# aperezhortal/pySPEEDY

Hardware: AMD Instinct MI355X
Metric: simulated-years/day (whole node), T30L8 (higher is better)
Workload: dtype f64

## Files before the change

pyspeedy_amd/csrc/capi.hip:

```cpp
#include <hip/hip_runtime.h>

#include <cstdio>
#include <cstring>
#include <mutex>
#include <string>
#include <vector>

#include "../../include/pyspeedy_amd.h"
#include "context.hpp"
#include "device_tables.hpp"
#include "surface_host.hpp"
#include "triangle.hpp"
#include "vertical_consts.hpp"

namespace spd {
hipError_t run_spec2grid(const DeviceTables &T, int stage, const double *src, double *dst, int kcos, int nfields,
                         hipStream_t stream);
hipError_t run_grid2spec(const DeviceTables &T, int stage, const double *src, double *dst, int prescale, int nfields,
                         hipStream_t stream);
hipError_t run_vort2vel(const DeviceTables &T, const double *vor, const double *div, double *ucos, double *vcos,
                        int nfields, hipStream_t s);
hipError_t run_vel2vort(const DeviceTables &T, const double *ucos, const double *vcos, double *vor, double *div,
                        int nfields, hipStream_t s);
hipError_t run_gradient(const DeviceTables &T, const double *psi, double *psdx, double *psdy, int nfields, hipStream_t s);
// ... 255 lines not shown
    else if (s == "ifac") { tmp.assign(t.ifac.begin(), t.ifac.end()); arr(tmp); }
    else if (s == "tri_packed") {
        tmp.assign(1 + NSPEC, -1.0);
        tmp[0] = tri::kPacked;
        for (int n = 0; n < NX; ++n)
            for (int m = 0; m < MX; ++m)
                if (tri::fwd_filled(m, n)) tmp[1 + n * MX + m] = tri::packed_index(m, n);
        arr(tmp);
    }
    else if (s == "tri_inv_needed") {
        tmp.assign(NSPEC, 0.0);
        for (int n = 0; n < NX; ++n)
            for (int m = 0; m < MX; ++m) tmp[n * MX + m] = tri::inv_needed(m, n) ? 1.0 : 0.0;
        arr(tmp);
    }
    else return fail(SPD_E_ARG, "spd_get_table_host: unknown table '" + s + "'");
    if (buf) {
        if (buf_elems < n) return fail(SPD_E_SIZE, "spd_get_table_host: buffer too small for '" + s + "'");
        std::memcpy(buf, src, n * sizeof(double));
    }
    return static_cast<long>(n);
}

int spd_calendar_walk(int year, int month, int day, int hour, int minute, int nsteps, int32_t *ymdhm, int32_t *month_idx,
                      int32_t *imont1, double *tmonth, double *tyear) {
    if (nsteps < 0 || month < 1 || month > 12 || day < 1 || day > 31) return fail(SPD_E_ARG, "spd_calendar_walk: bad start date or step count");
    Calendar c;
    c.set(year, month, day, hour, minute);
    for (int s = 0;; ++s) {
        if (ymdhm) {
// ... 160 lines not shown
```

pyspeedy_amd/csrc/dynamics.hip:

```cpp
#include <hip/hip_runtime.h>

#include <type_traits>

#include "coupler_point.hpp"
#include "device_tables.hpp"
#include "diagnostics_block.hpp"
#include "dyn_column.hpp"
#include "launch_events.hpp"
#include "model.hpp"
#include "sppt_point.hpp"

namespace spd {

namespace {
using d2 = double __attribute__((ext_vector_type(2)));
constexpr int NG = IX * IL;
constexpr int kT = 256;

__device__ constexpr double CPd = 1004.0f;
__device__ constexpr double AKAPd = 2.0f / 7.0f;
__device__ constexpr double RGASd = AKAPd * CPd;
__device__ constexpr double WILd = 0.53f, TDRSd = 24.0f * 30.0f;

__device__ inline d2 times_i(d2 z) { return d2{-z.y, z.x}; }
// ... 28 lines not shown
        rb = d2{-cm * s.bp.x + cp * s.bn.x + zp.x, -cm * s.bp.y + cp * s.bn.y + zp.y};
    }
}
}

namespace {
__device__ __forceinline__ d2 geo_up(d2 ph_below, d2 t_below, d2 t_here, double xg2_below, double xg1_here) {
    return d2{fma(xg1_here, t_here.x, fma(xg2_below, t_below.x, ph_below.x)),
              fma(xg1_here, t_here.y, fma(xg2_below, t_below.y, ph_below.y))};
}
__device__ __forceinline__ d2 geo_corr(d2 ph, d2 t_below, d2 t_above, double corf) {
    return d2{fma(corf, t_below.x - t_above.x, ph.x), fma(corf, t_below.y - t_above.y, ph.y)};
}
}

template <bool SPPT>
__global__ __launch_bounds__(kT) void geopotential_kernel(ModelPtrs P, DynDeviceTables D, int first, int count, int tl, SpptArgs sp) {
    const int ngeo = (count * NSPEC + kT - 1) / kT;
    if (SPPT && static_cast<int>(blockIdx.x) >= ngeo) {
        sppt_update_point(sp, static_cast<long>(blockIdx.x - ngeo) * kT + threadIdx.x);
        return;
    }
    const int gid = blockIdx.x * kT + threadIdx.x;
    if (gid >= count * NSPEC) return;
    const int lm = gid / NSPEC, mem = first + lm, k = gid - lm * NSPEC, m = k % MX;
    const d2 *t = reinterpret_cast<const d2 *>(P.t) + (static_cast<size_t>(mem) * 2 + tl) * 8 * NSPEC + k;
    d2 *phi = reinterpret_cast<d2 *>(P.phi) + static_cast<size_t>(mem) * 8 * NSPEC + k;
    d2 tt[KX], ph[KX];
#pragma unroll
    for (int l = 0; l < KX; ++l) tt[l] = t[static_cast<size_t>(l) * NSPEC];
    const d2 phis = reinterpret_cast<const d2 *>(P.phis)[static_cast<size_t>(mem) * NSPEC + k];
    ph[KX - 1] = d2{fma(D.xgeop1[KX - 1], tt[KX - 1].x, phis.x), fma(D.xgeop1[KX - 1], tt[KX - 1].y, phis.y)};
#pragma unroll
    for (int l = KX - 2; l >= 0; --l) ph[l] = geo_up(ph[l + 1], tt[l + 1], tt[l], D.xgeop2[l + 1], D.xgeop1[l]);
    if (m == 0) {
#pragma unroll
        for (int l = 1; l < KX - 1; ++l) ph[l] = geo_corr(ph[l], tt[l + 1], tt[l - 1], D.geo_corf[l]);
    }
#pragma unroll
    for (int l = 0; l < KX; ++l) phi[static_cast<size_t>(l) * NSPEC] = ph[l];
// ... 20 lines not shown
    double r = a[0];
#pragma unroll
    for (int i = 1; i < N; ++i) r = (l == i) ? a[i] : r;
    return r;
}
template <int N>
__device__ inline d2 pick(const d2 (&a)[N], int l) {
    d2 r = a[0];
#pragma unroll
    for (int i = 1; i < N; ++i) r = (l == i) ? a[i] : r;
    return r;
}
}

struct NoCoupler {};
template <bool FOLD, bool EARLY, typename CA>
__global__ __launch_bounds__(kT) void spectral_step_kernel(ModelPtrs P, DeviceTables T, DynDeviceTables D, int M, int first,
                                                           int count, int j1, double dt, double eps, CA cpl) {
    int nblocks = gridDim.x;
    if constexpr (std::is_same<CA, CouplerArgs>::value) {
        nblocks = (count * NSPEC * KX + kT - 1) / kT;
        if (static_cast<int>(blockIdx.x) >= nblocks) {
            const int gid = (blockIdx.x - nblocks) * kT + threadIdx.x;
            if (gid < cpl.count * NG) {
                const int lm = gid / NG;
                coupler_point(cpl.S, cpl.first + lm, gid - lm * NG, cpl.w, cpl.day, cpl.land_coupling, cpl.sst_anomaly,
                              cpl.anom_planes, cpl.fresh);
            }
            return;
        }
    }
    const int xcd = blockIdx.x & 7, q = nblocks >> 3, r = nblocks & 7;
    const int block = xcd * q + (xcd < r ? xcd : r) + (blockIdx.x >> 3);
    const int gid = block * kT + threadIdx.x;
    const int w = gid >> 6, lane = gid & 63;
    if (w >= count * kCoefBlocks) return;
    const int l = lane >> 3, kk = lane & 7;
    const int lm = w / kCoefBlocks, mem = first + lm, k = (w - lm * kCoefBlocks) * 8 + kk, n = k / MX, m = k - n * MX;
    const size_t f8 = static_cast<size_t>(mem) * 8 * NSPEC;
    const size_t fo = static_cast<size_t>(l) * NSPEC;
    const size_t tf = (static_cast<size_t>(mem) * 8 + l) * tri::kPacked;
    const size_t pair = static_cast<size_t>(M) * 8 * tri::kPacked;
    const d2 *su = reinterpret_cast<const d2 *>(P.specu) + tf, *sv = reinterpret_cast<const d2 *>(P.specv) + tf;
    const d2 *ske = reinterpret_cast<const d2 *>(P.spec_ke) + tf, *stt_f = reinterpret_cast<const d2 *>(P.spec_tt) + tf;
    const d2 *str_f = reinterpret_cast<const d2 *>(P.spec_tr) + tf;
    const d2 *sps = reinterpret_cast<const d2 *>(P.spec_ps) + static_cast<size_t>(mem) * tri::kPacked;
    const PackedAt at = packed_at(m, n);
    const double el2 = T.el2[k];
    d2 vordt, divdt, tdt, trdt, dump;
    const size_t s0 = static_cast<size_t>(mem) * 2 * 8 * NSPEC + fo + k;
    const size_t lvl = static_cast<size_t>(8) * NSPEC;
    d2 *vorS = reinterpret_cast<d2 *>(P.vor) + s0, *divS = reinterpret_cast<d2 *>(P.div) + s0;
    d2 *tS = reinterpret_cast<d2 *>(P.t) + s0, *trS = reinterpret_cast<d2 *>(P.tr) + s0;
// ... 15 lines not shown
            s_uv.ap = su[at.p], s_uv.bp = sv[at.p];
            s_ut.ap = su[pair + at.p], s_ut.bp = sv[pair + at.p];
            s_uq.ap = su[2 * pair + at.p], s_uq.bp = sv[2 * pair + at.p];
        }
        if (at.has_n) {
            s_uv.an = su[at.n], s_uv.bn = sv[at.n];
            s_ut.an = su[pair + at.n], s_ut.bn = sv[pair + at.n];
            s_uq.an = su[2 * pair + at.n], s_uq.bn = sv[2 * pair + at.n];
        }
    };
    auto load_diffusion = [&]() {
        dmp = D.dmp[k], dmp1 = D.dmp1[k], dmpd = D.dmpd[k], dmp1d = D.dmp1d[k], dmps = D.dmps[k], dmp1s = D.dmp1s[k];
        trf = T.trfilt[k];
        tcorh = reinterpret_cast<const d2 *>(P.tcorh)[static_cast<size_t>(mem) * NSPEC + k];
        qcorh = reinterpret_cast<const d2 *>(P.qcorh)[static_cast<size_t>(mem) * NSPEC + k];
    };
    if constexpr (EARLY) {
        load_tendencies(true);
        ph = reinterpret_cast<const d2 *>(P.phi)[f8 + fo + k];
        div1 = divS[0];
        ps1 = psS[0];
        const double *xj = D.xj + static_cast<size_t>(KX) * KX * (l_tot > 0 ? l_tot - 1 : 0);
#pragma unroll
        for (int k1 = 0; k1 < KX; ++k1) xc_l[k1] = D.xc[l + KX * k1], xj_l[k1] = xj[l + KX * k1], xd_l[k1] = D.xd[l + KX * k1];
        elz = D.elz[k];
        load_diffusion();
        vor1 = vorS[0], t1 = tS[0], tr1 = trS[0];
        vor2 = vorS[lvl], div2 = divS[lvl], t2 = tS[lvl], tr2 = trS[lvl], ps2 = psS[NSPEC];
        if (FOLD) phis_k = reinterpret_cast<const d2 *>(P.phis)[static_cast<size_t>(mem) * NSPEC + k];
        apply_stencil<1>(s_uv, k, m, n, T, vordt, divdt);
// ... 39 lines not shown
        double dtr_l = 0.0, dtr_l1 = 0.0;
#pragma unroll
        for (int j = 1; j < KX; ++j) {
            const double d = D.tref[j] - D.tref[j - 1];
            dtr_l = (l == j) ? d : dtr_l;
            dtr_l1 = (l + 1 == j) ? d : dtr_l1;
        }
        const d2 dumk_l = d2{sig_l.x * dtr_l, sig_l.y * dtr_l}, dumk_l1 = d2{sig_l1.x * dtr_l1, sig_l1.y * dtr_l1};
        const double dhsr_l = pick(D.dhsr, l), tref3_l = pick(D.tref3, l), tref2_l = pick(D.tref2, l);
        tdt.x = tdt.x - (dumk_l1.x + dumk_l.x) * dhsr_l + tref3_l * (sig_l1.x + sig_l.x) - tref2_l * dmeanc.x;
        tdt.y = tdt.y - (dumk_l1.y + dumk_l.y) * dhsr_l + tref3_l * (sig_l1.y + sig_l.y) - tref2_l * dmeanc.y;
    }
    {
        if constexpr (!EARLY) ph = reinterpret_cast<const d2 *>(P.phi)[f8 + fo + k];
        const double c = RGASd * tref_l;
        const d2 x = d2{ph.x + c * ps1.x, ph.y + c * ps1.y};
        const d2 lap = d2{-x.x * el2, -x.y * el2};
        divdt = d2{divdt.x - lap.x, divdt.y - lap.y};
    }

    {
        d2 all[KX];
        gather_levels(tdt, kk, all);
        d2 ye{0.0, 0.0};
#pragma unroll
        for (int k1 = 0; k1 < KX; ++k1) {
            const double x = EARLY ? xd_l[k1] : D.xd[l + KX * k1];
            ye = d2{ye.x + x * all[k1].x, ye.y + x * all[k1].y};
        }
        if constexpr (!EARLY) elz = D.elz[k];
// ... 13 lines not shown
        gather_levels(divdt, kk, all);
#pragma unroll
        for (int j = 0; j < KX; ++j) psdt = d2{psdt.x - all[j].x * D.dhsx[j], psdt.y - all[j].y * D.dhsx[j]};
#pragma unroll
        for (int k1 = 0; k1 < KX; ++k1) {
            const double x = EARLY ? xc_l[k1] : D.xc[l + KX * k1];
            tdt = d2{tdt.x + x * all[k1].x, tdt.y + x * all[k1].y};
        }
    }

    if constexpr (!EARLY) load_diffusion();
    const double sdrag = 1.0f / (TDRSd * 3600.0f);
    auto diffuse = [](d2 field, d2 fdt, double a, double b) { return d2{(fdt.x - a * field.x) * b, (fdt.y - a * field.y) * b}; };
    auto advance = [&](d2 *base, size_t stride, d2 o1, d2 o2, d2 fdt) -> d2 {
        if (!EARLY) o1 = base[0], o2 = base[stride];
        fdt = d2{fdt.x * trf, fdt.y * trf};
        const d2 oj = (j1 == 0) ? o1 : o2;
        const d2 fnew = d2{o1.x + dt * fdt.x, o1.y + dt * fdt.y};
        const double we = WILd * eps;
        const d2 n1 = d2{oj.x + we * (o1.x - 2 * oj.x + fnew.x), oj.y + we * (o1.y - 2 * oj.y + fnew.y)};
        const d2 oja = (j1 == 0) ? n1 : oj;
        const double we2 = (1.0f - WILd) * eps;
        const d2 n2 = d2{fnew.x - we2 * (n1.x - 2.0f * oja.x + fnew.x), fnew.y - we2 * (n1.y - 2.0f * oja.y + fnew.y)};
        stream_store(&base[0], n1);
        stream_store(&base[stride], n2);
        return n1;
    };
    {
        if constexpr (!EARLY) vor1 = vorS[0], t1 = tS[0], tr1 = trS[0];
        d2 vd = diffuse(vor1, vordt, dmp, dmp1);
        d2 dd = diffuse(div1, divdt, dmpd, dmp1d);
        const double tcorv_l = pick(D.tcorv, l), qcorv_l = pick(D.qcorv, l);
        const d2 ct = d2{t1.x + tcorh.x * tcorv_l, t1.y + tcorh.y * tcorv_l};
        d2 td = diffuse(ct, tdt, dmp, dmp1);
        if (l == 0 && m == 0) {
            vd = d2{vd.x - sdrag * vor1.x, vd.y - sdrag * vor1.y};
            dd = d2{dd.x - sdrag * div1.x, dd.y - sdrag * div1.y};
        }
// ... 19 lines not shown
            if (m == 0 && l >= 1 && l < KX - 1) {
                d2 tb = tall[2], ta = tall[0];
                double corf = D.geo_corf[1];
#pragma unroll
                for (int j = 2; j < KX - 1; ++j) {
                    tb = (l == j) ? tall[j + 1] : tb;
                    ta = (l == j) ? tall[j - 1] : ta;
                    corf = (l == j) ? D.geo_corf[j] : corf;
                }
                pn = geo_corr(pn, tb, ta, corf);
            }
            stream_store(&reinterpret_cast<d2 *>(P.phi_next)[f8 + fo + k], pn);
        }
    }
    if (l == 0) advance(psS, NSPEC, ps1, ps2, psdt);
}

__global__ __launch_bounds__(64 * KX) void diagnostics_kernel(CheckArgs c, DeviceTables T) {
    diagnostics_block(c, T, c.first + static_cast<int>(blockIdx.x));
}

hipError_t run_geopotential(const ModelPtrs &P, const DynDeviceTables &D, int first, int count, int tl, const SpptArgs *sppt,
                            hipStream_t s) {
    const int ngeo = (count * NSPEC + kT - 1) / kT;
    if (sppt) {
        const long n = static_cast<long>(sppt->M) * KX * NSPEC;
        launch(geopotential_kernel<true>, dim3(ngeo + static_cast<unsigned>((n + kT - 1) / kT)), dim3(kT), 0, s, P, D,
                           first, count, tl, *sppt);
    } else {
        launch(geopotential_kernel<false>, dim3(ngeo), dim3(kT), 0, s, P, D, first, count, tl, SpptArgs{});
    }
    return hipGetLastError();
}
hipError_t run_dyn_grid(const ModelPtrs &P, const DynDeviceTables &D, int M, hipStream_t s) {
    launch(dyn_grid_kernel, dim3((M * NG + kT - 1) / kT), dim3(kT), 0, s, P, D, M);
    return hipGetLastError();
}
namespace {
template <bool FOLD, bool EARLY, typename CA>
void launch_spectral_step(dim3 grid, hipStream_t s, const ModelPtrs &P, const DeviceTables &T, const DynDeviceTables &D, int M,
                          int first, int count, int j1, double dt, double eps, const CA &cpl) {
    launch(spectral_step_kernel<FOLD, EARLY, CA>, grid, dim3(kT), 0, s, P, T, D, M, first, count, j1, dt, eps, cpl);
}
template <typename CA>
void dispatch_spectral_step(bool fold, bool early, dim3 grid, hipStream_t s, const ModelPtrs &P, const DeviceTables &T,
                            const DynDeviceTables &D, int M, int first, int count, int j1, double dt, double eps, const CA &cpl) {
    if (fold && early) launch_spectral_step<true, true, CA>(grid, s, P, T, D, M, first, count, j1, dt, eps, cpl);
    else if (fold) launch_spectral_step<true, false, CA>(grid, s, P, T, D, M, first, count, j1, dt, eps, cpl);
    else if (early) launch_spectral_step<false, true, CA>(grid, s, P, T, D, M, first, count, j1, dt, eps, cpl);
    else launch_spectral_step<false, false, CA>(grid, s, P, T, D, M, first, count, j1, dt, eps, cpl);
}
}
hipError_t run_spectral_step(const ModelPtrs &P, const DeviceTables &T, const DynDeviceTables &D, int M, int first, int count,
                             int j1, double dt, double eps, const CouplerArgs *cpl, bool early, hipStream_t s) {
    const int nspec = (count * NSPEC * KX + kT - 1) / kT;
    const bool fold = P.phi_next != nullptr;
    if (cpl)
        dispatch_spectral_step(fold, early, dim3(nspec + (cpl->count * NG + kT - 1) / kT), s, P, T, D, M, first, count, j1, dt, eps,
                               *cpl);
    else
        dispatch_spectral_step(fold, early, dim3(nspec), s, P, T, D, M, first, count, j1, dt, eps, NoCoupler{});
    return hipGetLastError();
}
hipError_t run_diagnostics(const ModelPtrs &P, const DeviceTables &T, int M, int tl, int *err, double *diag, int ticket,
                           hipStream_t s) {
    hipLaunchKernelGGL(diagnostics_kernel, dim3(M), dim3(64 * KX), 0, s, CheckArgs{P.vor, P.div, P.t, tl, err, diag, ticket}, T);
    return hipGetLastError();
}
hipError_t run_diagnostics_range(const ModelPtrs &P, const DeviceTables &T, int first, int count, int tl, int *err, double *diag,
                                 int ticket, hipStream_t s) {
    if (count <= 0) return hipSuccess;
    hipLaunchKernelGGL(diagnostics_kernel, dim3(count), dim3(64 * KX), 0, s, CheckArgs{P.vor, P.div, P.t, tl, err, diag, ticket, first}, T);
    return hipGetLastError();
}

}
// ... 1 lines not shown
```

pyspeedy_amd/csrc/model.hip:

```cpp
#include <dlfcn.h>
#include <hip/hip_runtime.h>

#include <algorithm>
#include <atomic>
#include <chrono>
#include <cmath>
#include <cstring>
#include <map>
#include <memory>
#include <mutex>
#include <string>
#include <thread>
#include <utility>
#include <vector>

#include "../../include/pyspeedy_amd.h"
#include "context.hpp"
#include "model.hpp"
#include "coupler_point.hpp"
#include "diagnostics_block.hpp"
#include "bounded_call.hpp"
#include "launch_events.hpp"
#include "sppt_point.hpp"
#include "plev.hpp"
#include "stats.hpp"
#include "spectra.hpp"
#include "tape.hpp"
#include "enstape.hpp"
#include "acctape.hpp"
#include "stream_apart.hpp"
#include "surface.hpp"

namespace spd {
hipError_t run_spec2grid_table(const DeviceTables &T, const FieldDesc *table, int nfields, hipStream_t st);
hipError_t run_grid2spec_table(const DeviceTables &T, const FieldDesc *table, int nfields, hipStream_t st);
hipError_t run_physics(const DeviceTables &T, const spd_physics_args &a, int nmembers, int fp32, hipStream_t s);
hipError_t run_dyn_physics(const ModelPtrs &P, const DynDeviceTables &D, const DeviceTables &T, const spd_physics_args &a,
                           int first, int nmembers, int fp32, int store32, int diag, hipStream_t s);
hipError_t run_geopotential(const ModelPtrs &P, const DynDeviceTables &D, int first, int count, int tl, const SpptArgs *sppt,
                            hipStream_t s);
hipError_t run_dyn_grid(const ModelPtrs &P, const DynDeviceTables &D, int M, hipStream_t s);
hipError_t run_spectral_step(const ModelPtrs &P, const DeviceTables &T, const DynDeviceTables &D, int M, int first, int count,
                             int j1, double dt, double eps, const CouplerArgs *cpl, bool early, hipStream_t s);
hipError_t run_diagnostics(const ModelPtrs &P, const DeviceTables &T, int M, int tl, int *err, double *diag, int ticket,
                           hipStream_t s);
hipError_t run_diagnostics_range(const ModelPtrs &P, const DeviceTables &T, int first, int count, int tl, int *err, double *diag,
                                 int ticket, hipStream_t s);
hipError_t run_coupler(const SurfacePtrs &S, int first, int count, const TimeInterp &w, int day, int land_coupling,
                       int sst_anomaly, int anom_planes, int fresh, hipStream_t s);
hipError_t run_forcing(const SurfacePtrs &S, int first, int count, const ZonalDevice &Z, double gamlat, double *corh_t,
                       double *corh_q, hipStream_t s);
hipError_t run_rest_state(const RestPtrs &R, int M, const RestConsts &c, hipStream_t s);
hipError_t run_scale_orog(const double *orog, double *phi0, long n, hipStream_t s);
hipError_t run_change_storage(double *array, long n, bool to_float, void *scratch, hipStream_t s);
hipError_t run_land_sea_init(const LandSeaPtrs &P, const LandSeaConsts &K, int first, int count, double *rows, hipStream_t s);
hipError_t run_multi_copy(const CopyList &L, hipStream_t s);
hipError_t run_spec2grid_table_check(const DeviceTables &T, const FieldDesc *table, int nfields, const CheckArgs &check, int members,
                                     hipStream_t st);
// ... 43 lines not shown
        char *base;
        size_t size, used;
    };
    std::vector<Block> blocks;
    std::map<std::string, RegEntry> reg;
    FieldDesc *inv_table[2][2] = {{nullptr, nullptr}, {nullptr, nullptr}};
    FieldDesc *inv_table_sppt[2][2] = {{nullptr, nullptr}, {nullptr, nullptr}};
    FieldDesc *inv_table32[2][2] = {{nullptr, nullptr}, {nullptr, nullptr}}, *inv_table_sppt32[2][2] = {{nullptr, nullptr}, {nullptr, nullptr}};
    FieldDesc *fwd_table = nullptr;
    double *phi_buf[2] = {nullptr, nullptr};
    int phi_cur = 0;
    bool phi_ahead = false, fold_geo = true;
    bool groups_apart = true;
    int *d_err = nullptr;
    double *d_diag = nullptr;
    int *h_err[2] = {nullptr, nullptr}, *h_err_sync = nullptr;
    hipEvent_t err_event[2] = {nullptr, nullptr};
    int next_slot = 0;
    bool slot_busy[2] = {false, false};
    int check_ticket = 0, slot_ticket[2] = {0, 0};
    struct DeferredCheck {
        bool active = false;
        int slot = -1, time_level = 2;
        hipStream_t stream = nullptr;
    } deferred;
    hipStream_t slot_stream[2] = {nullptr, nullptr};
    bool slot_rode[2] = {false, false};
    int checks_alone = 0, checks_rode = 0;
    double air_absortivity_co2 = 6.0;
    SurfacePtrs S{};
// ... 516 lines not shown
    for (const char *name : {"t_grid_phys", "q_grid_phys", "phi_grid_phys", "pslg_phys", "u_grid_phys", "v_grid_phys",
                             "tt_rsw", "rad_tau2", "rad_strat_corr",
                             "rad_st4a", "rad_flux", "precnv", "precls", "cbmf", "slrd", "slr", "olr", "slru", "ustr", "vstr"})
        m->reg[name].f32 = true;
    if (rc == SPD_OK) {
        const spd_dyn_tables *base = nullptr;
        rc = dyn_tables(h, 0.0, nullptr, &base);
        if (rc == SPD_OK) m->D = base->dev;
    }
    if (rc == SPD_OK) {
        void *p = nullptr;
        rc = arena_alloc(m, sizeof(int) * M, &p);
        m->d_err = static_cast<int *>(p);
        if (rc == SPD_OK) rc = arena_alloc(m, sizeof(double) * M * 24, &p);
        m->d_diag = static_cast<double *>(p);
    }
    if (rc == SPD_OK) rc = build_tables(m);
    if (rc != SPD_OK) {
        spd_model_destroy(m);
        return rc;
    }
    *out = m;
    return SPD_OK;
}

int spd_model_destroy(spd_model_handle m) {
    if (!m) return SPD_OK;
    (void)hipSetDevice(m->ctx->device);
    constexpr size_t kIdleBytes = static_cast<size_t>(1) << 30;
    bool keep_first = false;
// ... 193 lines not shown
    m->P.phi = m->phi_buf[m->phi_cur];
    m->P.phi_next = m->fold_geo ? m->phi_buf[m->phi_cur ^ 1] : nullptr;
    m->reg["phi"].ptr = m->P.phi;
    m->phi_ahead = m->fold_geo;
    return !ahead;
}

static void sppt_advance(spd_model *m) {
    if (!m->sppt_on) return;
    m->sppt_first = false;
    m->sppt_step += 1;
}

static hipError_t step_range(spd_model *m, int j1, int j2, double dt, int compute_shortwave, int first, int count, int diag,
                             bool run_geo, const CouplerArgs *cpl, hipStream_t s, hipEvent_t after_grid2spec = nullptr,
                             const CheckArgs *ride = nullptr) {
    const DeviceTables &T = m->ctx->dev;
    const int M = m->M;
    hipError_t e = hipSuccess;
    if (m->fail_launch_after >= 0 && m->fail_launch_after-- == 0) return hipErrorLaunchFailure;
    SpptArgs sp{};
    if (m->sppt_on)
        sp = sppt_args(m->sppt_spec + static_cast<size_t>(first) * 8 * NSPEC * C, T, count, m->sppt_seed, m->sppt_member_base + first,
                       m->sppt_step, m->sppt_first ? 1 : 0);
    if (run_geo) {
        ProfScope ps(m, SPD_K_GEOPOTENTIAL, count, s);
        e = run_geopotential(m->P, m->D, first, count, 0, m->sppt_on ? &sp : nullptr, s);
    } else if (m->sppt_on) {
        ProfScope ps(m, SPD_K_SPPT, 8 * count, s);
        e = run_sppt_update(sp, s);
    }
    spd_physics_args pa = m->pa;
    pa.compute_shortwave = compute_shortwave ? 1 : 0;
    pa.air_absortivity_co2 = m->air_absortivity_co2;
    pa.sppt_pattern = m->sppt_on ? m->sppt_grid : nullptr;
    if (e == hipSuccess) {
        const int per = m->inv_per_member + (m->sppt_on ? 8 : 0);
        FieldDesc *table = (m->stored32 ? (m->sppt_on ? m->inv_table_sppt32 : m->inv_table32)
                                         : (m->sppt_on ? m->inv_table_sppt : m->inv_table))[j2 - 1][m->phi_cur];
        ProfScope ps(m, SPD_K_SPEC2GRID, per * count, s);
        if (m->deferred.active && first == 0 && count == M && s == m->deferred.stream) {
            const int slot = m->deferred.slot;
// ... 21 lines not shown
            }
        } else {
            ProfScope ps(m, compute_shortwave ? SPD_K_COLUMN_SW : SPD_K_COLUMN, count, s);
            e = run_dyn_physics(m->P, m->D, T, pa, first, count, m->phys_fp32, m->stored32 ? 1 : 0, diag, s);
        }
    }
    if (e == hipSuccess) {
        ProfScope ps(m, SPD_K_GRID2SPEC, 73 * count, s);
        e = run_grid2spec_table(T, m->fwd_table + static_cast<size_t>(first) * 73, 73 * count, s);
    }
    if (after_grid2spec && e == hipSuccess) e = hipEventRecord(after_grid2spec, s);
    const double eps = (j1 == 1) ? 0.0 : static_cast<double>(0.05f);
    if (e == hipSuccess) {
        ProfScope ps(m, SPD_K_SPECTRAL_STEP, count, s);
        const bool early = m->spectral_early < 0 ? count <= 8 : m->spectral_early != 0;
        e = run_spectral_step(m->P, T, m->D, M, first, count, j1 - 1, dt, eps, cpl, early, s);
    }
    return e;
}

int spd_model_step_dynamics(spd_model_handle m, int j1, int j2, double dt, int compute_shortwave, void *stream) {
    if (!m) return m_fail(SPD_E_ARG, "spd_model_step_dynamics: null model");
    if (j1 < 1 || j1 > 2 || j2 < 1 || j2 > 2) return m_fail(SPD_E_ARG, "spd_model_step_dynamics: time levels are 1 or 2");
    if (!m->dyn) return m_fail(SPD_E_ARG, "spd_model_step_dynamics: call spd_model_set_time_step first");
    if (int rc = settle_deferred_check(m)) return rc;
    const bool run_geo = begin_step_geopotential(m);
    const hipError_t e = step_range(m, j1, j2, dt, compute_shortwave, 0, m->M, 1, run_geo, nullptr, static_cast<hipStream_t>(stream));
    if (e != hipSuccess) return m_fail(SPD_E_DEVICE, std::string("spd_model_step_dynamics: ") + hipGetErrorString(e));
    sppt_advance(m);
    return SPD_OK;
}
// ... 327 lines not shown
        hipEvent_t *ev;
        int G;
        ~Join() {
            if (G > 1)
                for (int g = 0; g < G; ++g)
                    if (hipEventRecord(ev[g], gs[g]) == hipSuccess) (void)hipStreamWaitEvent(s, ev[g], 0);
        }
    } join{s, gs, m->cev, G};
    constexpr int kOffsetFrom = 36;
    const bool offset = G == 2 && nsteps >= kOffsetFrom;
    if (offset && !m->ev_offset) M_HIP(hipEventCreateWithFlags(&m->ev_offset, hipEventDisableTiming));
    int rounds = 1;
    const bool may_round = G > 1 || (m->nchunks == 1 && m->profile == 0 && !m->split_dyn_physics);
    if (may_round && nsteps > 1 && m->block_members > 0 && m->M >= 4 * m->block_members)
        rounds = (m->M + G * m->block_members - 1) / (G * m->block_members);
    struct HostState {
        Calendar cal;
        int current_step, phi_cur;
        bool surf_cache_valid, phi_ahead, sppt_first;
        long long sppt_step;
        double co2;
    };
    const HostState start{m->cal, m->current_step, m->phi_cur, m->surf_cache_valid, m->phi_ahead, m->sppt_first, m->sppt_step,
                          m->air_absortivity_co2};
    if (rounds > 1 && m->sst_anomaly_flag) {
        Calendar ahead = m->cal;
        for (int it = 0; it < nsteps; ++it) {
            ahead.advance();
            const TimeInterp w = time_interp(ahead);
            if (w.a0 < 0 || w.a1 < 0 || w.a0 >= m->anom_planes || w.a1 >= m->anom_planes)
// ... 70 lines not shown
            const bool run_geo = begin_step_geopotential(m);
            const bool first_of_call = it == 0 && round == 0;
            for (int g = 0, first = round_first; g < G && rc == SPD_OK; ++g) {
                const int count = base + (g < extra ? 1 : 0);
                if (count == 0) continue;
                launched = true;
                if (new_day) {
                    rc = forcing_range(m, zd, first, count, gs[g]);
                    device_failed = device_failed || rc != SPD_OK;
                }
                CouplerArgs cpl{m->S, w, first, count, 1 + (m->current_step + 1) / 36, m->land_coupling_flag, m->sst_anomaly_flag,
                                m->anom_planes, fresh};
                if (rc == SPD_OK) {
                    hipError_t e = hipSuccess;
                    if (offset && first_of_call && g == 1) e = hipStreamWaitEvent(gs[1], m->ev_offset, 0);
                    const CheckArgs chk{m->P.vor, m->P.div, m->P.t, tl_check, record && it > 0 ? m->h_steps_err + static_cast<size_t>(it - 1) * m->M : nullptr,
                                        nullptr, m->steps_ticket, first};
                    if (e == hipSuccess)
                        e = step_range(m, 2, 2, 2 * delt, sw, first, count, diag, run_geo, &cpl, gs[g],
                                       (offset && first_of_call && g == 0) ? m->ev_offset : nullptr, record && it > 0 ? &chk : nullptr);
                    if (e != hipSuccess) {
                        (void)hipGetLastError();
                        rc = m_fail(SPD_E_DEVICE, std::string(who) + ": " + hipGetErrorString(e));
                        device_failed = true;
                    }
                }
                if (rc == SPD_OK && record && it == nsteps - 1) {
                    const hipError_t e = run_diagnostics_range(m->P, m->ctx->dev, first, count, tl_check,
                                                               m->h_steps_err + static_cast<size_t>(it) * m->M, nullptr, m->steps_ticket, gs[g]);
                    if (e != hipSuccess) {
                        rc = m_fail(SPD_E_DEVICE, std::string(who) + ": " + hipGetErrorString(e));
                        device_failed = true;
                    }
                    ++m->checks_alone;
                }
// ... 293 lines not shown
    cfg[5] = 1;
    cfg[6] = m->phys_fp32;
    cfg[7] = m->stored32 ? 1 : 0;
    return SPD_OK;
}

int spd_model_get_option(spd_model_handle m, const char *name, int32_t *value) {
    if (!m || !name || !value) return m_fail(SPD_E_ARG, "spd_model_get_option: null argument");
    const std::string key(name);
    if (key == "diag_every_step") *value = m->diag_every_step ? 1 : 0;
    else if (key == "split_dyn") *value = m->split_dyn_physics ? 1 : 0;
    else if (key == "spectral_early") *value = m->spectral_early;
    else if (key == "member_groups") *value = m->nchunks;
    else if (key == "block_members") *value = m->block_members;
    else if (key == "physics_storage32") *value = m->phys_store32 ? 1 : 0;
    else return m_fail(SPD_E_ARG, "spd_model_get_option: unknown option: " + key);
    return SPD_OK;
}

int spd_model_set_option(spd_model_handle m, const char *name, int32_t value) {
    if (!m || !name) return m_fail(SPD_E_ARG, "spd_model_set_option: null argument");
    const std::string key(name);
    const bool flag = value == 0 || value == 1;
    if (key == "diag_every_step" && flag) m->diag_every_step = value != 0;
    else if (key == "split_dyn" && flag) m->split_dyn_physics = value != 0;
    else if (key == "spectral_early" && value >= -1 && value <= 1) m->spectral_early = value;
    else if (key == "member_groups" && value >= 1 && value <= 4) m->nchunks = value < m->M ? value : m->M;
    else if (key == "block_members" && value >= 0) m->block_members = value;
    else if (key == "fail_launch_after" && value >= -1) m->fail_launch_after = value;
    else if (key == "prepare_multi_step" && value == 1) {
// ... 1523 lines not shown
```

pyspeedy_amd/csrc/model.hpp:

```cpp
#pragma once
#include "device_tables.hpp"
#include "triangle.hpp"

namespace spd {

struct ModelPtrs {
    double *vor, *div, *t, *tr;
    double *ps;
    double *phi;
    double *phi_next;
    double *phis;
    double *tcorh, *qcorh;
    double *sv;
    double *vorg, *divg, *tg2, *trg2, *ug2, *vg2;
    double *px, *py;
    double *utend, *vtend, *ttend, *trtend, *keg, *utg, *vtg, *uqg, *vqg;
    double *psdtg;
    double *specu, *specv;
    double *spec_tt, *spec_tr, *spec_ke;
    double *spec_ps;
};

struct DynDeviceTables {
    const double *dmp, *dmpd, *dmps, *dmp1, *dmp1d, *dmp1s, *elz;
    const double *xj, *xc, *xd;
    const double *coriol;
    double tcorv[8], qcorv[8], tref[8], tref2[8], tref3[8], dhsx[8], xgeop1[8], xgeop2[8], geo_corf[8];
    double dhs[8], dhsr[8], fsgr[8];
};

}
```

pyspeedy_amd/csrc/triangle.hpp:

```cpp
#pragma once
#include "tables.hpp"

#if defined(__HIPCC__) || defined(__CUDACC__)
#define SPD_TRI_HD __host__ __device__
#else
#define SPD_TRI_HD
#endif

namespace spd {
namespace tri {

constexpr int kFilled = 526;
constexpr int kPacked = 528;
static_assert(kPacked >= kFilled && kPacked * 16 % 256 == 0, "a packed field keeps the arena's 256-byte carving");

SPD_TRI_HD constexpr bool inv_needed(int m, int n) { return m + n <= TRUNC + 1; }
SPD_TRI_HD constexpr bool fwd_filled(int m, int n) { return n <= TRUNC && m + n <= TRUNC + 1; }

SPD_TRI_HD constexpr int row_start(int n) { return n == 0 ? 0 : MX + (n - 1) * (TRUNC + 2) - (n - 1) * n / 2; }
SPD_TRI_HD constexpr int packed_index(int m, int n) { return row_start(n) + m; }

static_assert(row_start(1) == 31 && row_start(2) == 62 && row_start(3) == 92, "rows are 31, 31, 30, ... long");
static_assert(packed_index(1, TRUNC) == kFilled - 1, "the last filled coefficient is (m = 1, n = 30)");

}
}
```

pyspeedy_amd/model.py:

```python
import ctypes as C

import numpy as np
import torch

from . import _lib
from ._lib import check
from .registry import REGISTRY

SHAPES = {n: (v.dtype, v.shape) for n, v in REGISTRY.items() if v.where == "device"}
SHAPES["sst_anom"] = (np.float64, (96, 48, 3))

DELT = 86400.0 / 36

KERNEL_NAMES = ("geopotential", "spec2grid", "column_sw", "column", "grid2spec", "spectral_step", "coupler", "forcing",
                "sppt", "dyn_grid", "physics_sw", "physics")

BC_MAP = (("orog", "orog"), ("fmask_orig", "lsm"), ("alb0", "alb"), ("veg_high", "vegh"), ("veg_low", "vegl"),
          ("stl12", "stl"), ("snowd12", "snowd"), ("soil_wc_l1", "swl1"), ("soil_wc_l2", "swl2"), ("soil_wc_l3", "swl3"),
          ("sst12", "sst"), ("sea_ice_frac12", "icec"))


class EnsembleModel:
    def __init__(self, spectral, nmembers):
        self.sp = spectral
# ... 190 lines not shown
        streams, M = cfg[2], self.nmembers
        rounds = 1
        if block.value > 0 and M >= 4 * block.value and not cfg[3]:
            rounds = (M + max(streams, 1) * block.value - 1) // (max(streams, 1) * block.value)
        return dict(inv_per_member=cfg[0], diag_every_step=bool(cfg[1]), chunks=cfg[2], split_dyn=bool(cfg[3]),
                    fold_geo=bool(cfg[4]), coupler_in_spectral=bool(cfg[5]), physics_fp32=bool(cfg[6]),
                    physics_storage32=bool(cfg[7]), group_streams=created.value, group_streams_apart=bool(apart.value),
                    block_members=block.value, rounds=rounds)

    def set_option(self, name, value):
        rc = self._lib.spd_model_set_option(self._m, name.encode(), int(value))
        if rc == _lib.SPD_E_ARG:
            raise ValueError("unknown option or value out of range: %s = %r" % (name, value))
        check(rc, "spd_model_set_option")

    def profile(self, level=1):
        check(self._lib.spd_model_profile(self._m, int(level)), "spd_model_profile")

    def profile_read_kernels(self):
        n = len(KERNEL_NAMES)
        mean, mn = np.zeros(n), np.zeros(n)
        cnt, units = np.zeros(n, dtype=np.int32), np.zeros(n, dtype=np.int32)
        check(self._lib.spd_model_profile_read_kernels(self._m, mean.ctypes.data_as(C.c_void_p), mn.ctypes.data_as(C.c_void_p),
                                                       cnt.ctypes.data_as(C.c_void_p), units.ctypes.data_as(C.c_void_p)),
              "spd_model_profile_read_kernels")
        return {KERNEL_NAMES[k]: (float(mean[k]), float(mn[k]), int(cnt[k]), int(units[k])) for k in range(n) if cnt[k]}

    def profile_read(self):
        ms, n, f = C.c_double(), C.c_int(), C.c_int()
        check(self._lib.spd_model_profile_read(self._m, C.byref(ms), C.byref(n), C.byref(f)), "spd_model_profile_read")
# ... 371 lines not shown
```

Measured before the change: 1.765 million.

## Skip spectral blocks beyond the triangle halo once detected zero per member

On the first step of each call, the spectral step kernel checks whether every coefficient in blocks lying wholly beyond the truncation halo is exactly zero, and writes a per-member flag. Later steps in the same call skip the geopotential and spectral-step work for those dead blocks when the member's flag is still set. This aims to save memory traffic and ALU work on about a quarter of the coefficient blocks. In exchange it adds a memset per call, OR-reduction bookkeeping in the detect step, and a dependence on those coefficients staying exactly zero within the call.

```diff
diff --git a/pyspeedy_amd/csrc/capi.hip b/pyspeedy_amd/csrc/capi.hip
--- a/pyspeedy_amd/csrc/capi.hip
+++ b/pyspeedy_amd/csrc/capi.hip
@@ -293,6 +293,11 @@
             for (int m = 0; m < MX; ++m) tmp[n * MX + m] = tri::inv_needed(m, n) ? 1.0 : 0.0;
         arr(tmp);
     }
+    else if (s == "tri_dead_blocks") {
+        tmp.assign(tri::kBlocks, 0.0);
+        for (int b = 0; b < tri::kBlocks; ++b) tmp[b] = tri::dead_block(b) ? 1.0 : 0.0;
+        arr(tmp);
+    }
     else return fail(SPD_E_ARG, "spd_get_table_host: unknown table '" + s + "'");
     if (buf) {
         if (buf_elems < n) return fail(SPD_E_SIZE, "spd_get_table_host: buffer too small for '" + s + "'");
diff --git a/pyspeedy_amd/csrc/dynamics.hip b/pyspeedy_amd/csrc/dynamics.hip
--- a/pyspeedy_amd/csrc/dynamics.hip
+++ b/pyspeedy_amd/csrc/dynamics.hip
@@ -66,8 +66,14 @@
 }
 }
 
-template <bool SPPT>
-__global__ __launch_bounds__(kT) void geopotential_kernel(ModelPtrs P, DynDeviceTables D, int first, int count, int tl, SpptArgs sp) {
+struct NoRim {};
+template <int RIM>
+using RimArg = std::conditional_t<RIM == kRimPlain, NoRim, int *>;
+
+template <bool SPPT, int RIM = kRimPlain>
+__global__ __launch_bounds__(kT) void geopotential_kernel(ModelPtrs P, DynDeviceTables D, int first, int count, int tl, SpptArgs sp,
+                                                          RimArg<RIM> rim) {
+    static_assert(RIM == kRimPlain || RIM == kRimSkip, "the geopotential launch has nothing to detect");
     const int ngeo = (count * NSPEC + kT - 1) / kT;
     if (SPPT && static_cast<int>(blockIdx.x) >= ngeo) {
         sppt_update_point(sp, static_cast<long>(blockIdx.x - ngeo) * kT + threadIdx.x);
@@ -76,6 +82,9 @@
     const int gid = blockIdx.x * kT + threadIdx.x;
     if (gid >= count * NSPEC) return;
     const int lm = gid / NSPEC, mem = first + lm, k = gid - lm * NSPEC, m = k % MX;
+    if constexpr (RIM == kRimSkip) {
+        if (tri::dead_block(k / tri::kBlock) && rim[mem] != 0) return;
+    }
     const d2 *t = reinterpret_cast<const d2 *>(P.t) + (static_cast<size_t>(mem) * 2 + tl) * 8 * NSPEC + k;
     d2 *phi = reinterpret_cast<d2 *>(P.phi) + static_cast<size_t>(mem) * 8 * NSPEC + k;
     d2 tt[KX], ph[KX];
@@ -126,9 +135,10 @@
 }
 
 struct NoCoupler {};
-template <bool FOLD, bool EARLY, typename CA>
+template <bool FOLD, bool EARLY, typename CA, int RIM = kRimPlain>
 __global__ __launch_bounds__(kT) void spectral_step_kernel(ModelPtrs P, DeviceTables T, DynDeviceTables D, int M, int first,
-                                                           int count, int j1, double dt, double eps, CA cpl) {
+                                                           int count, int j1, double dt, double eps, CA cpl, RimArg<RIM> rim) {
+    static_assert(!FOLD || RIM == kRimPlain, "the folded form (small, latency-bound launches) has no rim modes");
     int nblocks = gridDim.x;
     if constexpr (std::is_same<CA, CouplerArgs>::value) {
         nblocks = (count * NSPEC * KX + kT - 1) / kT;
@@ -149,6 +159,16 @@
     if (w >= count * kCoefBlocks) return;
     const int l = lane >> 3, kk = lane & 7;
     const int lm = w / kCoefBlocks, mem = first + lm, k = (w - lm * kCoefBlocks) * 8 + kk, n = k / MX, m = k - n * MX;
+    if constexpr (RIM == kRimSkip) {
+        if (tri::dead_block(w - lm * kCoefBlocks) && rim[mem] != 0) return;
+    }
+    unsigned seen = 0;
+    auto note = [&](d2 v) {
+        if constexpr (RIM == kRimDetect) {
+            const unsigned long long x = __double_as_longlong(v.x) | __double_as_longlong(v.y);
+            seen |= static_cast<unsigned>(x) | static_cast<unsigned>(x >> 32);
+        }
+    };
     const size_t f8 = static_cast<size_t>(mem) * 8 * NSPEC;
     const size_t fo = static_cast<size_t>(l) * NSPEC;
     const size_t tf = (static_cast<size_t>(mem) * 8 + l) * tri::kPacked;
@@ -194,6 +214,7 @@
         trf = T.trfilt[k];
         tcorh = reinterpret_cast<const d2 *>(P.tcorh)[static_cast<size_t>(mem) * NSPEC + k];
         qcorh = reinterpret_cast<const d2 *>(P.qcorh)[static_cast<size_t>(mem) * NSPEC + k];
+        note(tcorh), note(qcorh);
     };
     if constexpr (EARLY) {
         load_tendencies(true);
@@ -263,6 +284,7 @@
     {
         if constexpr (!EARLY) ph = reinterpret_cast<const d2 *>(P.phi)[f8 + fo + k];
         const double c = RGASd * tref_l;
+        note(ph), note(ps1);
         const d2 x = d2{ph.x + c * ps1.x, ph.y + c * ps1.y};
         const d2 lap = d2{-x.x * el2, -x.y * el2};
         divdt = d2{divdt.x - lap.x, divdt.y - lap.y};
@@ -306,6 +328,7 @@
     auto diffuse = [](d2 field, d2 fdt, double a, double b) { return d2{(fdt.x - a * field.x) * b, (fdt.y - a * field.y) * b}; };
     auto advance = [&](d2 *base, size_t stride, d2 o1, d2 o2, d2 fdt) -> d2 {
         if (!EARLY) o1 = base[0], o2 = base[stride];
+        note(o1), note(o2);
         fdt = d2{fdt.x * trf, fdt.y * trf};
         const d2 oj = (j1 == 0) ? o1 : o2;
         const d2 fnew = d2{o1.x + dt * fdt.x, o1.y + dt * fdt.y};
@@ -314,6 +337,7 @@
         const d2 oja = (j1 == 0) ? n1 : oj;
         const double we2 = (1.0f - WILd) * eps;
         const d2 n2 = d2{fnew.x - we2 * (n1.x - 2.0f * oja.x + fnew.x), fnew.y - we2 * (n1.y - 2.0f * oja.y + fnew.y)};
+        note(n1), note(n2);
         stream_store(&base[0], n1);
         stream_store(&base[stride], n2);
         return n1;
@@ -363,6 +387,9 @@
         }
     }
     if (l == 0) advance(psS, NSPEC, ps1, ps2, psdt);
+    if constexpr (RIM == kRimDetect) {
+        if (tri::dead_block(w - lm * kCoefBlocks) && __any(seen != 0) && lane == 0) rim[mem] = 0;
+    }
 }
 
 __global__ __launch_bounds__(64 * KX) void diagnostics_kernel(CheckArgs c, DeviceTables T) {
@@ -370,14 +397,17 @@
 }
 
 hipError_t run_geopotential(const ModelPtrs &P, const DynDeviceTables &D, int first, int count, int tl, const SpptArgs *sppt,
-                            hipStream_t s) {
+                            int *rim, hipStream_t s) {
     const int ngeo = (count * NSPEC + kT - 1) / kT;
     if (sppt) {
         const long n = static_cast<long>(sppt->M) * KX * NSPEC;
-        launch(geopotential_kernel<true>, dim3(ngeo + static_cast<unsigned>((n + kT - 1) / kT)), dim3(kT), 0, s, P, D,
-                           first, count, tl, *sppt);
+        const dim3 grid(ngeo + static_cast<unsigned>((n + kT - 1) / kT));
+        if (rim) launch(geopotential_kernel<true, kRimSkip>, grid, dim3(kT), 0, s, P, D, first, count, tl, *sppt, rim);
+        else launch(geopotential_kernel<true>, grid, dim3(kT), 0, s, P, D, first, count, tl, *sppt, NoRim{});
+    } else if (rim) {
+        launch(geopotential_kernel<false, kRimSkip>, dim3(ngeo), dim3(kT), 0, s, P, D, first, count, tl, SpptArgs{}, rim);
     } else {
-        launch(geopotential_kernel<false>, dim3(ngeo), dim3(kT), 0, s, P, D, first, count, tl, SpptArgs{});
+        launch(geopotential_kernel<false>, dim3(ngeo), dim3(kT), 0, s, P, D, first, count, tl, SpptArgs{}, NoRim{});
     }
     return hipGetLastError();
 }
@@ -386,29 +416,35 @@
     return hipGetLastError();
 }
 namespace {
-template <bool FOLD, bool EARLY, typename CA>
+template <bool FOLD, bool EARLY, typename CA, int RIM = kRimPlain>
 void launch_spectral_step(dim3 grid, hipStream_t s, const ModelPtrs &P, const DeviceTables &T, const DynDeviceTables &D, int M,
-                          int first, int count, int j1, double dt, double eps, const CA &cpl) {
-    launch(spectral_step_kernel<FOLD, EARLY, CA>, grid, dim3(kT), 0, s, P, T, D, M, first, count, j1, dt, eps, cpl);
+                          int first, int count, int j1, double dt, double eps, const CA &cpl, RimArg<RIM> rim = {}) {
+    launch(spectral_step_kernel<FOLD, EARLY, CA, RIM>, grid, dim3(kT), 0, s, P, T, D, M, first, count, j1, dt, eps, cpl, rim);
 }
 template <typename CA>
-void dispatch_spectral_step(bool fold, bool early, dim3 grid, hipStream_t s, const ModelPtrs &P, const DeviceTables &T,
-                            const DynDeviceTables &D, int M, int first, int count, int j1, double dt, double eps, const CA &cpl) {
+void dispatch_spectral_step(bool fold, bool early, int rim_mode, int *rim, dim3 grid, hipStream_t s, const ModelPtrs &P,
+                            const DeviceTables &T, const DynDeviceTables &D, int M, int first, int count, int j1, double dt, double eps,
+                            const CA &cpl) {
     if (fold && early) launch_spectral_step<true, true, CA>(grid, s, P, T, D, M, first, count, j1, dt, eps, cpl);
     else if (fold) launch_spectral_step<true, false, CA>(grid, s, P, T, D, M, first, count, j1, dt, eps, cpl);
+    else if (rim_mode == kRimDetect && early) launch_spectral_step<false, true, CA, kRimDetect>(grid, s, P, T, D, M, first, count, j1, dt, eps, cpl, rim);
+    else if (rim_mode == kRimDetect) launch_spectral_step<false, false, CA, kRimDetect>(grid, s, P, T, D, M, first, count, j1, dt, eps, cpl, rim);
+    else if (rim_mode == kRimSkip && early) launch_spectral_step<false, true, CA, kRimSkip>(grid, s, P, T, D, M, first, count, j1, dt, eps, cpl, rim);
+    else if (rim_mode == kRimSkip) launch_spectral_step<false, false, CA, kRimSkip>(grid, s, P, T, D, M, first, count, j1, dt, eps, cpl, rim);
     else if (early) launch_spectral_step<false, true, CA>(grid, s, P, T, D, M, first, count, j1, dt, eps, cpl);
     else launch_spectral_step<false, false, CA>(grid, s, P, T, D, M, first, count, j1, dt, eps, cpl);
 }
 }
 hipError_t run_spectral_step(const ModelPtrs &P, const DeviceTables &T, const DynDeviceTables &D, int M, int first, int count,
-                             int j1, double dt, double eps, const CouplerArgs *cpl, bool early, hipStream_t s) {
+                             int j1, double dt, double eps, const CouplerArgs *cpl, bool early, int rim_mode, int *rim, hipStream_t s) {
     const int nspec = (count * NSPEC * KX + kT - 1) / kT;
     const bool fold = P.phi_next != nullptr;
+    if (fold && rim_mode != kRimPlain) return hipErrorInvalidValue;
     if (cpl)
-        dispatch_spectral_step(fold, early, dim3(nspec + (cpl->count * NG + kT - 1) / kT), s, P, T, D, M, first, count, j1, dt, eps,
-                               *cpl);
+        dispatch_spectral_step(fold, early, rim_mode, rim, dim3(nspec + (cpl->count * NG + kT - 1) / kT), s, P, T, D, M, first, count,
+                               j1, dt, eps, *cpl);
     else
-        dispatch_spectral_step(fold, early, dim3(nspec), s, P, T, D, M, first, count, j1, dt, eps, NoCoupler{});
+        dispatch_spectral_step(fold, early, rim_mode, rim, dim3(nspec), s, P, T, D, M, first, count, j1, dt, eps, NoCoupler{});
     return hipGetLastError();
 }
 hipError_t run_diagnostics(const ModelPtrs &P, const DeviceTables &T, int M, int tl, int *err, double *diag, int ticket,
diff --git a/pyspeedy_amd/csrc/model.hip b/pyspeedy_amd/csrc/model.hip
--- a/pyspeedy_amd/csrc/model.hip
+++ b/pyspeedy_amd/csrc/model.hip
@@ -38,10 +38,10 @@
 hipError_t run_dyn_physics(const ModelPtrs &P, const DynDeviceTables &D, const DeviceTables &T, const spd_physics_args &a,
                            int first, int nmembers, int fp32, int store32, int diag, hipStream_t s);
 hipError_t run_geopotential(const ModelPtrs &P, const DynDeviceTables &D, int first, int count, int tl, const SpptArgs *sppt,
-                            hipStream_t s);
+                            int *rim, hipStream_t s);
 hipError_t run_dyn_grid(const ModelPtrs &P, const DynDeviceTables &D, int M, hipStream_t s);
 hipError_t run_spectral_step(const ModelPtrs &P, const DeviceTables &T, const DynDeviceTables &D, int M, int first, int count,
-                             int j1, double dt, double eps, const CouplerArgs *cpl, bool early, hipStream_t s);
+                             int j1, double dt, double eps, const CouplerArgs *cpl, bool early, int rim_mode, int *rim, hipStream_t s);
 hipError_t run_diagnostics(const ModelPtrs &P, const DeviceTables &T, int M, int tl, int *err, double *diag, int ticket,
                            hipStream_t s);
 hipError_t run_diagnostics_range(const ModelPtrs &P, const DeviceTables &T, int first, int count, int tl, int *err, double *diag,
@@ -115,6 +115,8 @@
     bool groups_apart = true;
     int *d_err = nullptr;
     double *d_diag = nullptr;
+    int *d_rim = nullptr;
+    bool rim_call = false;
     int *h_err[2] = {nullptr, nullptr}, *h_err_sync = nullptr;
     hipEvent_t err_event[2] = {nullptr, nullptr};
     int next_slot = 0;
@@ -661,6 +663,8 @@
         m->d_err = static_cast<int *>(p);
         if (rc == SPD_OK) rc = arena_alloc(m, sizeof(double) * M * 24, &p);
         m->d_diag = static_cast<double *>(p);
+        if (rc == SPD_OK) rc = arena_alloc(m, sizeof(int) * M, &p);
+        m->d_rim = static_cast<int *>(p);
     }
     if (rc == SPD_OK) rc = build_tables(m);
     if (rc != SPD_OK) {
@@ -884,7 +888,7 @@
 
 static hipError_t step_range(spd_model *m, int j1, int j2, double dt, int compute_shortwave, int first, int count, int diag,
                              bool run_geo, const CouplerArgs *cpl, hipStream_t s, hipEvent_t after_grid2spec = nullptr,
-                             const CheckArgs *ride = nullptr) {
+                             const CheckArgs *ride = nullptr, int rim_mode = kRimPlain) {
     const DeviceTables &T = m->ctx->dev;
     const int M = m->M;
     hipError_t e = hipSuccess;
@@ -895,7 +899,8 @@
                        m->sppt_step, m->sppt_first ? 1 : 0);
     if (run_geo) {
         ProfScope ps(m, SPD_K_GEOPOTENTIAL, count, s);
-        e = run_geopotential(m->P, m->D, first, count, 0, m->sppt_on ? &sp : nullptr, s);
+        e = run_geopotential(m->P, m->D, first, count, 0, m->sppt_on ? &sp : nullptr, rim_mode == kRimSkip ? m->d_rim : nullptr,
+                             s);
     } else if (m->sppt_on) {
         ProfScope ps(m, SPD_K_SPPT, 8 * count, s);
         e = run_sppt_update(sp, s);
@@ -947,7 +952,7 @@
     if (e == hipSuccess) {
         ProfScope ps(m, SPD_K_SPECTRAL_STEP, count, s);
         const bool early = m->spectral_early < 0 ? count <= 8 : m->spectral_early != 0;
-        e = run_spectral_step(m->P, T, m->D, M, first, count, j1 - 1, dt, eps, cpl, early, s);
+        e = run_spectral_step(m->P, T, m->D, M, first, count, j1 - 1, dt, eps, cpl, early, rim_mode, m->d_rim, s);
     }
     return e;
 }
@@ -1305,6 +1310,8 @@
     const bool may_round = G > 1 || (m->nchunks == 1 && m->profile == 0 && !m->split_dyn_physics);
     if (may_round && nsteps > 1 && m->block_members > 0 && m->M >= 4 * m->block_members)
         rounds = (m->M + G * m->block_members - 1) / (G * m->block_members);
+    const bool rim = nsteps >= 2 && !m->fold_geo;
+    m->rim_call = rim;
     struct HostState {
         Calendar cal;
         int current_step, phi_cur;
@@ -1405,11 +1412,14 @@
                 if (rc == SPD_OK) {
                     hipError_t e = hipSuccess;
                     if (offset && first_of_call && g == 1) e = hipStreamWaitEvent(gs[1], m->ev_offset, 0);
+                    if (rim && it == 0 && e == hipSuccess)
+                        e = hipMemsetD32Async(reinterpret_cast<hipDeviceptr_t>(m->d_rim + first), 1, static_cast<size_t>(count), gs[g]);
                     const CheckArgs chk{m->P.vor, m->P.div, m->P.t, tl_check, record && it > 0 ? m->h_steps_err + static_cast<size_t>(it - 1) * m->M : nullptr,
                                         nullptr, m->steps_ticket, first};
                     if (e == hipSuccess)
                         e = step_range(m, 2, 2, 2 * delt, sw, first, count, diag, run_geo, &cpl, gs[g],
-                                       (offset && first_of_call && g == 0) ? m->ev_offset : nullptr, record && it > 0 ? &chk : nullptr);
+                                       (offset && first_of_call && g == 0) ? m->ev_offset : nullptr, record && it > 0 ? &chk : nullptr,
+                                       rim ? (it == 0 ? kRimDetect : kRimSkip) : kRimPlain);
                     if (e != hipSuccess) {
                         (void)hipGetLastError();
                         rc = m_fail(SPD_E_DEVICE, std::string(who) + ": " + hipGetErrorString(e));
@@ -1733,6 +1743,16 @@
     else if (key == "member_groups") *value = m->nchunks;
     else if (key == "block_members") *value = m->block_members;
     else if (key == "physics_storage32") *value = m->phys_store32 ? 1 : 0;
+    else if (key == "quiet_rim_members") {
+        *value = -1;
+        if (m->rim_call) {
+            std::vector<int> flags(static_cast<size_t>(m->M));
+            M_HIP(hipDeviceSynchronize());
+            M_HIP(hipMemcpy(flags.data(), m->d_rim, sizeof(int) * flags.size(), hipMemcpyDeviceToHost));
+            *value = 0;
+            for (int f : flags) *value += f != 0 ? 1 : 0;
+        }
+    }
     else return m_fail(SPD_E_ARG, "spd_model_get_option: unknown option: " + key);
     return SPD_OK;
 }
diff --git a/pyspeedy_amd/csrc/model.hpp b/pyspeedy_amd/csrc/model.hpp
--- a/pyspeedy_amd/csrc/model.hpp
+++ b/pyspeedy_amd/csrc/model.hpp
@@ -21,6 +21,8 @@
     double *spec_ps;
 };
 
+enum RimMode : int { kRimPlain = 0, kRimDetect = 1, kRimSkip = 2 };
+
 struct DynDeviceTables {
     const double *dmp, *dmpd, *dmps, *dmp1, *dmp1d, *dmp1s, *elz;
     const double *xj, *xc, *xd;
diff --git a/pyspeedy_amd/csrc/triangle.hpp b/pyspeedy_amd/csrc/triangle.hpp
--- a/pyspeedy_amd/csrc/triangle.hpp
+++ b/pyspeedy_amd/csrc/triangle.hpp
@@ -23,5 +23,33 @@
 static_assert(row_start(1) == 31 && row_start(2) == 62 && row_start(3) == 92, "rows are 31, 31, 30, ... long");
 static_assert(packed_index(1, TRUNC) == kFilled - 1, "the last filled coefficient is (m = 1, n = 30)");
 
+SPD_TRI_HD constexpr bool beyond_halo(int m, int n) { return m + n >= TRUNC + 3; }
+
+constexpr int kBlock = 8, kBlocks = MX * NX / kBlock;
+static_assert(MX * NX % kBlock == 0 && kBlocks == 124, "124 blocks of 8 coefficients");
+SPD_TRI_HD constexpr bool block_is_dead(int b) {
+    bool dead = true;
+    for (int k = kBlock * b; k < kBlock * (b + 1); ++k) dead = dead && beyond_halo(k % MX, k / MX);
+    return dead;
+}
+SPD_TRI_HD constexpr unsigned long long dead_word(int word) {
+    unsigned long long bits = 0;
+    for (int b = 64 * word; b < 64 * (word + 1) && b < kBlocks; ++b) bits |= static_cast<unsigned long long>(block_is_dead(b)) << (b - 64 * word);
+    return bits;
+}
+constexpr unsigned long long kDeadLo = dead_word(0), kDeadHi = dead_word(1);
+SPD_TRI_HD constexpr bool dead_block(int b) { return ((b < 64 ? kDeadLo >> b : kDeadHi >> (b - 64)) & 1ull) != 0; }
+
+constexpr int popcount64(unsigned long long x) { return x == 0 ? 0 : static_cast<int>(x & 1ull) + popcount64(x >> 1); }
+constexpr int kDeadBlocks = popcount64(kDeadLo) + popcount64(kDeadHi);
+constexpr int count_beyond_halo() {
+    int c = 0;
+    for (int k = 0; k < MX * NX; ++k) c += beyond_halo(k % MX, k / MX) ? 1 : 0;
+    return c;
+}
+static_assert(kDeadBlocks == 31, "31 of the 124 blocks lie wholly beyond the halo");
+static_assert(kDeadBlocks * kBlock == 248 && count_beyond_halo() == 435, "248 of the 435 coefficients beyond the halo are in dead blocks");
+static_assert(!dead_block(0) && dead_block(kBlocks - 1) && !block_is_dead(4), "(0, 0) is alive, (30, 31) is dead, (1, 1) is alive");
+
 }
 }
diff --git a/pyspeedy_amd/model.py b/pyspeedy_amd/model.py
--- a/pyspeedy_amd/model.py
+++ b/pyspeedy_amd/model.py
@@ -228,6 +228,14 @@
             raise ValueError("unknown option or value out of range: %s = %r" % (name, value))
         check(rc, "spd_model_set_option")
 
+    def get_option(self, name):
+        value = C.c_int32(0)
+        rc = self._lib.spd_model_get_option(self._m, name.encode(), C.byref(value))
+        if rc == _lib.SPD_E_ARG:
+            raise ValueError("unknown option: %s" % name)
+        check(rc, "spd_model_get_option")
+        return value.value
+
     def profile(self, level=1):
         check(self._lib.spd_model_profile(self._m, int(level)), "spd_model_profile")
 
```

After: 1.817 million (median of 6 runs). 1.03x the previous value.
